# tyb311/TCCT

Measured on AMD Instinct MI355X. Metric: OCT B-scans/sec fwd+bwd(+clip+AdamW), stc_tt bs=8 1x800x1100, higher is better.
Workload: dtype bf16; 1 GPU; stc_tt --los=di bs=8/GPU 1x800x1100 (net tensors 3x800x1104); global_batch=8, parallelism=dp1, ranks=1, grad_allreduce=none, slowest_step=101

## Files before the change

### include/tcct_hip.h

```cpp
#ifndef TCCT_HIP_H
#define TCCT_HIP_H
#include <stdint.h>
#ifdef __cplusplus
extern "C" {
#endif

typedef void* tcct_stream_t;

enum { TCCT_F32 = 0, TCCT_BF16 = 1 };
enum { TCCT_ACT_NONE = 0, TCCT_ACT_LRELU = 1, TCCT_ACT_HSWISH = 2, TCCT_ACT_GELU = 3, TCCT_ACT_SIGMOID = 4,
       TCCT_ACT_ABS = 5 };

int tcct_version(void);
const char* tcct_last_error(void);
int tcct_set_outputs_prezeroed(int on);

int tcct_image_to_nhwc4(const float* img, void* out, int N, int Csrc, int H, int Wsrc, int Wdst, int dtype,
                        tcct_stream_t stream);
int tcct_u8_gather2d(const uint8_t* src, uint8_t* dst, int N, int SH, int SW, int C, int sy0, int sx0, int sh, int sw, int DH, int DW,
                     int dy0, int dx0, int dh, int dw, int flipy, int flipx, int mul, int div, int fill, tcct_stream_t stream);
int tcct_onehot_to_index(const int64_t* onehot, uint8_t* lab, int N, int C, int64_t HW, tcct_stream_t stream);
int tcct_labels_to_u8(const int64_t* lab, uint8_t* out, int N, int H, int Wsrc, int Wdst, tcct_stream_t stream);
int tcct_nhwc_to_nchw_f32(const void* x, float* y, int N, int64_t HW, int C, int dtype, tcct_stream_t stream);

// ... 50 lines not shown
int tcct_bn2_add_act_train(const void* xa, const void* xb, void* y, int64_t M, int C, const double* sumsA, const float* gammaA,
                           const float* betaA, float* running_meanA, float* running_varA, int64_t* nbtA, float* mean_rstdA,
                           float* abA, const double* sumsB, const float* gammaB, const float* betaB, float* running_meanB,
                           float* running_varB, int64_t* nbtB, float* mean_rstdB, float* abB, float eps, float momentum,
                           int pre_act, int act, int dtype, tcct_stream_t stream);
int tcct_bn2_add_act_bwd_reduce(const void* xa, const void* xb, const void* dy, int64_t M, int C, const float* mean_rstdA,
                                const float* abA, const float* mean_rstdB, const float* abB, int pre_act, int act, double* sums,
                                int dtype, tcct_stream_t stream);
int tcct_bn2_add_act_bwd_apply(const void* xa, const void* xb, const void* dy, void* dxa, void* dxb, int64_t M, int C,
                               const float* mean_rstdA, const float* abA, const float* mean_rstdB, const float* abB,
                               const double* sums, int pre_act, int act, float* dgammaA, float* dbetaA, float* dgammaB,
                               float* dbetaB, int dtype, tcct_stream_t stream);

int tcct_layernorm_fwd(const void* x, void* y, int64_t M, int C, const float* gamma, const float* beta, float eps,
                       float* mean_rstd , int dtype, tcct_stream_t stream);
int tcct_layernorm_bwd(const void* x, const void* dy, void* dx, int64_t M, int C, const float* gamma,
                       const float* mean_rstd, float* dgamma, float* dbeta, int dtype, tcct_stream_t stream);
int tcct_layernorm_bwd_add(const void* x, const void* dy, const void* res, void* dx, int64_t M, int C, const float* gamma,
                           const float* mean_rstd, float* dgamma, float* dbeta, int dtype, tcct_stream_t stream);

int tcct_conv2d_fwd(const void* x, const float* w, const float* bias, void* y, int N, int H, int W, int Cin,
                    int Cin_w, int Cout, int KH, int KW, int stride, int padh, int padw, int in_dtype, int out_dtype,
                    tcct_stream_t stream);
int tcct_conv2d_dgrad(const void* dy, const float* w, void* dx, int N, int H, int W, int Cin, int Cout, int KH,
                      int KW, int padh, int padw, int dy_dtype, int dx_dtype, tcct_stream_t stream);
int tcct_conv2d_wgrad(const void* x, const void* dy, float* dw, float* dbias, int N, int H, int W, int Cin,
                      int Cin_w, int Cout, int KH, int KW, int stride, int padh, int padw, int x_dtype, int dy_dtype,
                      tcct_stream_t stream);

int tcct_conv32f_pack_weights(const float* w, float* wp, int KH, int KW, int transposed, tcct_stream_t stream);
int tcct_conv32f_fwd(const float* x, const float* wp, const float* bias, const float* yadd, float* y, int N, int H, int W, int KH, int KW, int PH,
                     int PW, tcct_stream_t stream);
int tcct_conv32f_wgrad(const float* x, const float* dy, float* dw, float* dbias, int N, int H, int W, int KH, int KW, int PH, int PW,
                       tcct_stream_t stream);
int tcct_conv32f_pack_weights_sub(const float* w, float* wp, int KH, int KW, int transposed, int cin_total, int o_off, int i_off, tcct_stream_t stream);
int tcct_conv32f_fwd_strided(const float* x, const float* wp, const float* bias, float* y, int N, int H, int W, int KH, int KW, int PH, int PW, int xs,
                             int xo, int ys, int yo, int accumulate, tcct_stream_t stream);
int tcct_conv32f_wgrad_strided(const float* x, const float* dy, float* dw, float* dbias, int N, int H, int W, int KH, int KW, int PH, int PW, int xs,
                               int xo, int ds, int dof, int ldi, int o_off, int i_off, tcct_stream_t stream);
int tcct_pwf_fwd(const float* x, const float* w, const float* bias, float* y, int64_t M, int K, int N, int transposed, tcct_stream_t stream);
int tcct_pwf_wgrad(const float* x, const float* dy, float* dw, float* dbias, int64_t M, int K, int N, tcct_stream_t stream);
int tcct_conv32_pack_weights(const float* w, void* wp, int KH, int KW, int transposed, tcct_stream_t stream);
int tcct_conv32_pack_weights_multi(const void* desc, int n, tcct_stream_t stream);
int tcct_conv32_pack_weights_both(const float* w, void* wp2, int KH, int KW, tcct_stream_t stream);
int tcct_conv32_fwd(const void* x, const void* wp, const float* bias, void* y, int N, int H, int W, int KH, int KW, int PH,
                    int PW, tcct_stream_t stream);

int tcct_conv32_fwd_bnstats(const void* x, const void* wp, const float* bias, void* y, int N, int H, int W, int KH, int KW, int PH,
                            int PW, double* stats, int pre_act, tcct_stream_t stream);
int tcct_conv32_fwd_affine(const void* x, const void* wp, const float* bias, void* y, int N, int H, int W, int KH, int KW,
                           int PH, int PW, const float* ab, int pre_act, int post_act, tcct_stream_t stream);
int tcct_pw_fwd_affine(const void* x, const float* w, const float* bias, void* y, int64_t M, int K, int N, const float* ab,
                       int pre_act, int post_act, int out_dtype, tcct_stream_t stream);
int tcct_pw_fwd_affine_residual(const void* x, const float* w, const float* bias, const float* ab, const void* res, void* y, int64_t M, int K, int N,
                                tcct_stream_t stream);
int tcct_pw_fwd_cat2_affine(const void* x1, const void* x2, const float* w, const float* bias, const float* ab, int post_act, void* y, int64_t M, int K, int N,
                            tcct_stream_t stream);
int tcct_pw_fwd_xaff_affine_residual(const void* y_prev, const float* ab_prev, const float* w, const float* bias, const float* ab, const void* res, void* y,
                                     int64_t M, int K, int N, tcct_stream_t stream);
int tcct_conv32_fwd_add(const void* x, const void* wp, const float* bias, const void* res, void* y, int N, int H, int W, int KH, int KW,
                        int PH, int PW, tcct_stream_t stream);
int tcct_conv32_chain33(const void* x, const void* wp1, const float* bias1, void* mid, const void* wp2, const float* bias2, void* y,
                        const void* res, int N, int H, int W, double* stats, tcct_stream_t stream);
int tcct_conv32_pack_weights_sub(const float* w, void* wp, int KH, int KW, int transposed, int cin_total, int o_off, int i_off,
                                 tcct_stream_t stream);
int tcct_conv32_fwd_strided(const void* x, const void* wp, const float* bias, void* y, int N, int H, int W, int KH, int KW, int PH,
                            int PW, int xs, int xo, int ys, int yo, int accumulate, tcct_stream_t stream);
int tcct_conv32_fwd_strided_bnstats(const void* x, const void* wp, const float* bias, void* y, int N, int H, int W, int KH, int KW, int PH,
                                    int PW, int xs, int xo, int ys, int yo, int accumulate, double* stats, int pre_act, tcct_stream_t stream);
int tcct_conv32_fwd_strided_affine(const void* x, const void* wp, const float* bias, void* y, int N, int H, int W, int KH, int KW, int PH, int PW, int xs,
                                   int xo, int ys, int yo, const float* ab, int pre_act, int post_act, tcct_stream_t stream);
int64_t tcct_conv32_wgrad_mode(int mode);
int64_t tcct_conv32_fwd_mode(int mode);
int tcct_conv32_wgrad_strided(const void* x, const void* dy, float* dw, float* dbias, int N, int H, int W, int KH, int KW, int PH,
                              int PW, int xs, int xo, int ds, int dof, int cin_total, int o_off, int i_off, tcct_stream_t stream);
int tcct_conv32_wgrad(const void* x, const void* dy, float* dw, float* dbias, int N, int H, int W, int KH, int KW, int PH,
                      int PW, tcct_stream_t stream);
int tcct_conv32_bwd3x3(const void* x, const void* dy, const void* wp_t, const void* dskip, void* dx, float* dw, float* dbias, int N, int H,
                       int W, tcct_stream_t stream);

int tcct_pw_fwd(const void* x, const float* w, const float* bias, void* y, int64_t M, int K, int N, int transposed,
                int out_dtype, tcct_stream_t stream);
int tcct_pw_wgrad(const void* x, const void* dy, float* dw, float* dbias, int64_t M, int K, int N, tcct_stream_t stream);
int tcct_pw_bwd(const void* x, const void* dy, const float* w, const void* res, void* dx, float* dw, float* dbias, int64_t M, int K, int N,
                tcct_stream_t stream);
int tcct_pw_bwd_cat2(const void* x1, const void* x2, const void* dy, const float* w, void* dx1, void* dx2, float* dw, int64_t M, int K, int N,
                     tcct_stream_t stream);
int tcct_pw_bwd_residual2(const void* x, const void* dy, const float* w, const void* res, void* dx_sum, void* dx_plain, float* dw, float* dbias,
                          int64_t M, int K, int N, tcct_stream_t stream);
int64_t tcct_pw_bwd_bn_supported(int K, int N, int post, int red_post, int split);
int tcct_pw_bwd_bn(const void* x, const void* x2, const void* dz, const void* y, const float* coef, int post, const float* w, const void* res,
                   void* dx, void* dx2, float* dw, float* dbias, int64_t M, int K, int N, const void* y_prev, const float* ab_prev,
                   int red_post, double* sums_prev, tcct_stream_t stream);
int tcct_pw_bwd_bn_sums(const void* x, const void* x2, const void* dz, const void* y, const double* sums, int raw, const float* mean_rstd,
                        const float* ab, float* dgamma, float* dbeta, int post, const float* w, const void* res, void* dx, void* dx2, float* dw,
                        float* dbias, int64_t M, int K, int N, const void* y_prev, const float* ab_prev, int red_post, double* sums_prev,
                        tcct_stream_t stream);
int tcct_pw_wgrad_strided(const void* x, const void* dy, int64_t ldy, float* dw, float* dbias, int64_t M, int K, int N,
                          tcct_stream_t stream);
int tcct_pw_fwd_residual(const void* x, const float* w, const float* bias, const void* res, const float* scale, int64_t per_sample,
                         void* y, void* y_plain, int64_t M, int K, int N, tcct_stream_t stream);
int tcct_pw_fwd_bnstats_xaff(const void* y_prev, const float* ab_prev, const float* w, const float* bias, void* y, int64_t M, int K, int N, double* stats,
                             tcct_stream_t stream);
int tcct_pw_bwd_bn_sums_xaff(const void* y_prev, const float* ab_prev, const void* dz, const void* y, const double* sums, int raw, const float* mean_rstd,
                             const float* ab, float* dgamma, float* dbeta, const float* w, const void* res, void* dx, float* dw, float* dbias, int64_t M,
                             int K, int N, int red_post, double* sums_prev, tcct_stream_t stream);
int tcct_pw_fwd_gelu_residual(const void* x1, const float* w, const float* bias, const void* res, const float* scale, int64_t per_sample, void* y,
                              int64_t M, int K, int N, tcct_stream_t stream);
int tcct_pw_bwd_residual2_sum(const void* x, const void* dy_a, const void* dy_b, const float* w, const void* res, void* dx_sum, void* dx_plain, float* dw,
                              float* dbias, int64_t M, int K, int N, tcct_stream_t stream);
int tcct_pw_bwd_lnb(const void* x, const void* dy, const float* w, const void* t, const float* mean_rstd, const float* gamma, const void* res, void* dt,
                    float* dw, float* dbias, float* dgamma, float* dbeta, int64_t M, int K, int N, tcct_stream_t stream);
int tcct_pw_bwd_gelu(const void* x1, const void* dy, const float* w, void* dx1, float* dw, float* dbias, int64_t M, int K, int N, tcct_stream_t stream);
int tcct_pw_dgrad_residual(const void* dy, const float* w, const void* res, void* dx_sum, void* dx_plain, int64_t M, int Nout, int K,
                           tcct_stream_t stream);
int tcct_pw_fwd_cat2(const void* x1, const void* x2, int K1, const float* w, const float* bias, void* y, int64_t M, int K, int N,
                     double* stats, int pre_act, tcct_stream_t stream);
int tcct_pw_fwd_f32_upadd(const void* x, const float* w, const float* bias, float* y, int B, int uH, int uW, int K, int N, const float* up, tcct_stream_t stream);
int tcct_pw_dgrad_split2(const void* dy, const float* w, void* dx1, void* dx2, int K1, int64_t M, int Nout, int K, tcct_stream_t stream);
int tcct_pw_bwd_cat2_bias(const void* x1, const void* x2, const void* dy, const float* w, void* dx1, void* dx2, float* dw, float* dbias, int64_t M,
                          int K, int N, tcct_stream_t stream);
int tcct_tail_compose(const float* w1, const float* b1, const float* w2, const float* b2, float* wc, float* c, tcct_stream_t stream);
int tcct_tail_compose_bwd(const float* w1, const float* b1, const float* w2, const float* dwc, const float* dc, float* dw1, float* db1, float* dw2,
                          float* db2, tcct_stream_t stream);
int tcct_tail_compose3(const float* w1, const float* b1, const float* w2, const float* b2, const float* w3, const float* b3, int C, float* wcc, float* wa,
                       float* wb, float* ccc, tcct_stream_t stream);
int tcct_tail_compose3_bwd(const float* w1, const float* b1, const float* w2, const float* b2, const float* w3, int C, const float* dwa, const float* dwb,
                           const float* dccc, float* dw1, float* db1, float* dw2, float* db2, float* dw3, float* db3, tcct_stream_t stream);
int tcct_pw_fwd_cat2_f32(const void* x1, const void* x2, int K1, const float* w, const float* bias, float* y, int64_t M, int K, int N, tcct_stream_t stream);
int tcct_head_compose(const float* wt, const float* bt, const float* wa, const float* ba, int C, float* wh, float* ch, tcct_stream_t stream);
int tcct_head_compose_bwd(const float* wt, const float* bt, const float* wa, int C, const float* dwh, const float* dch, float* dwt, float* dbt,
                          float* dwa, float* dba, tcct_stream_t stream);
int tcct_pw_wgrad_cat2(const void* x1, const void* x2, int K1, const void* dy, float* dw, float* dbias, int64_t M, int K, int N,
                       tcct_stream_t stream);
int tcct_pw_fwd_bnstats(const void* x, const float* w, const float* bias, void* y, int64_t M, int K, int N, double* stats, int pre_act,
                        tcct_stream_t stream);

int tcct_im2col3x3_c3(const void* x4, void* out, int N, int H, int W, int stride, int dtype, tcct_stream_t stream);
int tcct_c3_fwd(const void* x4, const float* w, const float* bias, void* y, int B, int H, int W, int stride, double* stats, int stat_pre,
                const float* ab, int pre_act, int post_act, tcct_stream_t stream);
int tcct_c3_wgrad(const void* x4, const void* dy, float* dw, float* dbias, int B, int H, int W, int stride, tcct_stream_t stream);
int tcct_c3_bn_fwd_train(const void* x4, const float* w, const float* bias, void* z, int B, int H, int W, int stride, double* sums,
                         const float* gamma, const float* beta, float eps, float momentum, float* running_mean, float* running_var,
                         int64_t* num_batches_tracked, float* mean_rstd, float* ab, int post_act, tcct_stream_t stream);
int tcct_c3_bn_fwd_eval(const void* x4, const float* w, const float* bias, void* z, int B, int H, int W, int stride, const float* ab, int post_act,
                        tcct_stream_t stream);
int tcct_c3_bn_bwd_reduce(const void* x4, const float* w, const float* bias, const void* dz, int B, int H, int W, int stride, const float* ab,
                          double* raw, int post_act, tcct_stream_t stream);
int tcct_c3_bn_bwd_wgrad(const void* x4, const float* w, const float* bias, const void* dz, int B, int H, int W, int stride, const float* coef,
                         float* dw, float* dbias, int post_act, tcct_stream_t stream);
int64_t tcct_c3_bn_bwd_prefetch(int tiles_ahead);
int tcct_c3_bn_bwd_onepass(const void* x4, const float* w, const float* bias, const void* dz, int B, int H, int W, int stride, const float* mean_rstd,
                           const float* ab, float* work, double* sums, float* dw, float* dbias, float* dgamma, float* dbeta, int post_act, tcct_stream_t stream);
int tcct_pw_wgrad_smalln(const void* x, const void* dy, float* dw, float* dbias, int64_t M, int K, int N, int x_dtype,
                         int dy_dtype, tcct_stream_t stream);

int tcct_stream_copy(const void* src, void* dst, int64_t nbytes, tcct_stream_t stream);

int64_t tcct_kernel_census(int which, int reset);
int tcct_marker(int id, tcct_stream_t stream);

int tcct_dwconv3x3_fwd(const void* x, const float* w, const float* bias, void* y, int N, int H, int W, int C,
                       int stride, int add_input, int dtype, tcct_stream_t stream);
int tcct_dwconv3x3_fwd_bnstats(const void* x, const float* w, const float* bias, void* y, int N, int H, int W, int C, int stride,
                               int add_input, double* stats, int dtype, tcct_stream_t stream);
int tcct_dwconv3x3_dgrad(const void* dy, const float* w, void* dx, int N, int H, int W, int C, int stride,
// ... 123 lines not shown
```

### tcct_amd/_lib.py

```python
import ctypes
import threading
import os
import re

import torch

_HERE = os.path.dirname(os.path.abspath(__file__))
LIB_PATH = os.path.join(_HERE, 'csrc', 'libtcct_hip.so')
if os.environ.get('TCCT_LIB_PATH'):
    LIB_PATH = os.path.abspath(os.environ['TCCT_LIB_PATH'])
HEADER = os.path.join(_HERE, '..', 'include', 'tcct_hip.h')

F32, BF16 = 0, 1
ACT_NONE, ACT_LRELU, ACT_HSWISH, ACT_GELU, ACT_SIGMOID, ACT_ABS = range(6)

_CT = {'int': ctypes.c_int, 'int64_t': ctypes.c_int64, 'float': ctypes.c_float, 'double': ctypes.c_double,
       'uint64_t': ctypes.c_uint64}


def parse_header(path=HEADER):
    src = open(path).read()
    src = re.sub(r'/\*.*?\*/', ' ', src, flags=re.S)
    src = re.sub(r'//[^\n]*', ' ', src)
    protos = {}
    for m in re.finditer(r'(const\s+char\s*\*|int64_t|int)\s+(tcct_\w+)\s*\(([^)]*)\)\s*;', src):
        ret, name, args = m.group(1), m.group(2), m.group(3).strip()
        sig = []
        if args and args != 'void':
            for a in args.split(','):
                a = ' '.join(a.split())
                if '*' in a or a.startswith('tcct_stream_t'):
                    sig.append((ctypes.c_void_p, a.split()[-1].lstrip('*')))
                else:
                    ty, nm = a.rsplit(' ', 1)
                    sig.append((_CT[ty.replace('const ', '').strip()], nm))
        protos[name] = (ctypes.c_char_p if 'char' in ret else (ctypes.c_int64 if 'int64' in ret else ctypes.c_int), sig)
    return protos


class TcctError(RuntimeError):
    pass


_TLS = threading.local()
_TRACE = [None]


class launch_on:

    def __init__(self, stream):
        self.handle = stream.cuda_stream

    def __enter__(self):
        self.prev = getattr(_TLS, 'stream', None)
        _TLS.stream = self.handle
        return self

    def __exit__(self, *exc):
        _TLS.stream = self.prev
        return False


class _Lib:
    def __init__(self):
        self._dll = None
        self.protos = parse_header()

    def load(self):
        if self._dll is None:
            if not os.path.exists(LIB_PATH):
                raise TcctError(f'{LIB_PATH} is missing: run `python -c "import __graft_entry__ as g; g.build()"` '
                                '(tcct_amd has no CPU fallback)')
            dll = ctypes.CDLL(LIB_PATH)
            for name, (res, sig) in self.protos.items():
                fn = getattr(dll, name)
                fn.restype = res
                fn.argtypes = [t for t, _ in sig]
            self._dll = dll
        return self._dll

    def last_error(self):
        return self.load().tcct_last_error().decode()

    def __getattr__(self, name):
        full = 'tcct_' + name
        if full not in self.protos:
            raise AttributeError(name)
        dll = self.load()
        fn = getattr(dll, full)
        sig = self.protos[full][1]
        res_is_value = self.protos[full][0] is not ctypes.c_int

        n = len(sig)
        has_stream = bool(sig) and sig[-1][1] == 'stream'
        is_ptr = tuple(ct is ctypes.c_void_p for ct, _ in sig)
        raw_stream, cur_dev, Tensor = torch._C._cuda_getCurrentRawStream, torch._C._cuda_getDevice, torch.Tensor

        tls, trace = _TLS, _TRACE

        def call(*args):
            if has_stream and len(args) == n - 1:
                args = args + (getattr(tls, 'stream', None) or raw_stream(cur_dev()),)
            elif len(args) != n:
                raise TypeError(f'{full}: expected {n} args ({[nm for _, nm in sig]}), got {len(args)}')
            if has_stream and trace[0] is not None:
                trace[0](full, sig, args)
            rc = fn(*[(a.data_ptr() if isinstance(a, Tensor) else a) if p and a is not None else a for a, p in zip(args, is_ptr)])
            if res_is_value:
                return rc
            if rc != 0:
                raise TcctError(f'{full} failed (rc={rc}): {dll.tcct_last_error().decode()}')
        call.__name__ = full
        self.__dict__[name] = call
        return call


lib = _Lib()


def dtype_code(t):
    if t == torch.float32:
        return F32
    if t == torch.bfloat16:
        return BF16
    raise TcctError(f'unsupported activation dtype {t}')
```

### tcct_amd/csrc/pw_mfma.hip

```cpp
#include "common.h"
#include "c3_geom.h"
#include <cstdlib>

typedef __attribute__((ext_vector_type(8))) __bf16 bf16x8;
typedef __attribute__((ext_vector_type(16))) float f32x16;
typedef __attribute__((ext_vector_type(4))) short s16x4;
typedef __attribute__((ext_vector_type(8))) short s16x8;
typedef __attribute__((__vector_size__(4 * sizeof(unsigned int)))) unsigned int u32x4;

#define PWB 256

__device__ __forceinline__ void st_out4(bf16* p, float a, float b, float c, float d) {
    uint2 o; o.x = pack_bf16x2(a, b); o.y = pack_bf16x2(c, d);
    *reinterpret_cast<uint2*>(p) = o;
}
__device__ __forceinline__ void st_out4(float* p, float a, float b, float c, float d) {
    *reinterpret_cast<float4*>(p) = make_float4(a, b, c, d);
}

__device__ __forceinline__ float rnd_out(float v, const bf16*) { return __bfloat162float(__float2bfloat16(v)); }
__device__ __forceinline__ float rnd_out(float v, const float*) { return v; }

struct PwUp { const float* p; int uH, uW, Ho, Wo; float sh, sw; uint32_t m_howo, m_wo; };
struct PwSplit { const bf16* x2; int K1; void* y2; int N1; const bf16* res; const float* rscale; int64_t per_sample; bf16* yplain; C3Geom c3; PwUp up; };
// ... 541 lines not shown
        return __builtin_bit_cast(bf16x8, v);
    };
    struct WF { bf16x8 a[NT], b[KTB]; };
    auto load_chunk = [&](WF& f, int ch) {
#pragma unroll
        for (int ct = 0; ct < NT; ++ct) f.a[ct] = tr2(lbD + ch * 16 * SD + 64 * ct, SD);
#pragma unroll
        for (int kt = 0; kt < KTB; ++kt) f.b[kt] = tr2(lbX + ch * 16 * SX + 64 * kt, SX);
    };
    auto mma_chunk = [&](const WF& f) {
        if (blockIdx.y == 0) {
#pragma unroll
            for (int ct = 0; ct < NT; ++ct)
#pragma unroll
                for (int j = 0; j < 8; ++j) bsum[ct] += (float)f.a[ct][j];
        }
#pragma unroll
        for (int kt = 0; kt < KTB; ++kt)
#pragma unroll
            for (int ct = 0; ct < NT; ++ct) acc[ct][kt] = __builtin_amdgcn_mfma_f32_32x32x16_bf16(f.a[ct], f.b[kt], acc[ct][kt], 0, 0, 0);
    };
    const int64_t tiles = (M + PW_P - 1) / PW_P;
    int64_t tile = blockIdx.x;
    if (C3)
        for (int i = tid; i < PW_P * 2; i += PWB) *reinterpret_cast<uint4*>(sX + (i >> 1) * SX + (6 + (i & 1)) * 16) = make_uint4(0, 0, 0, 0);
    if (tile < tiles) prefetch(tile);
    for (; tile < tiles; tile += gridDim.x) {
        __syncthreads();
        if (C3) {
#pragma unroll
            for (int j = 0; j < 3; ++j)
                if (xsl[j] >= 0) *reinterpret_cast<uint4*>(sX + (tid & 127) * SX + (xsl[j] & 255) * 16) = px[j];
        } else
#pragma unroll
        for (int j = 0; j < PW_XS; ++j)
            if (xsl[j] >= 0) *reinterpret_cast<uint4*>(sX + (xsl[j] >> 8) * SX + (xsl[j] & 255) * 16) = px[j];
#pragma unroll
        for (int j = 0; j < DSN; ++j)
            if (dsl[j] >= 0) *reinterpret_cast<uint4*>(sD + (dsl[j] >> 8) * SD + (dsl[j] & 255) * 16) = pd[j];
        __syncthreads();
        if (C3 || tile + gridDim.x < tiles) prefetch(tile + gridDim.x);
        WF f0, f1;
        load_chunk(f0, wave);
        load_chunk(f1, wave + 4);
        __builtin_amdgcn_sched_barrier(0);
        mma_chunk(f0);
        mma_chunk(f1);
        __builtin_amdgcn_sched_barrier(0);
    }
    __syncthreads();
    float* red = reinterpret_cast<float*>(smem);
    for (int turn = 0; turn < 4; ++turn) {
        if (wave == turn) {
#pragma unroll
            for (int ct = 0; ct < NT; ++ct)
#pragma unroll
                for (int kt = 0; kt < KTB; ++kt)
#pragma unroll
                    for (int k = 0; k < 16; ++k) {
                        const int co = ct * 32 + (k & 3) + 8 * (k >> 2) + 4 * hh;
                        float* dst = &red[co * (KTB * 32) + kt * 32 + r];
                        *dst = turn == 0 ? acc[ct][kt][k] : *dst + acc[ct][kt][k];
                    }
        }
        __syncthreads();
    }
    for (int i = tid; i < NT * 32 * KTB * 32; i += PWB) {
        const int co = i / (KTB * 32), cl = i - co * (KTB * 32);
        if (C3) {
            if (cl < 48 && ((cl >> 2) & 3) < 3 && (cl & 3) < 3) atomicAdd(&dw[co * 27 + (cl & 3) * 9 + (cl >> 4) * 3 + ((cl >> 2) & 3)], red[i]);
        }
        else
        if (co < N && ci_base + cl < K) atomicAdd(&dw[(int64_t)co * K + ci_base + cl], red[i]);
    }
    if (dbias && blockIdx.y == 0) {
#pragma unroll
        for (int ct = 0; ct < NT; ++ct) {
            float s = bsum[ct] + __shfl_xor(bsum[ct], 32, 64);
            if (lane < 32 && ct * 32 + r < N) atomicAdd(&dbias[ct * 32 + r], s);
        }
    }
}

static int pw_wgrad_impl(const void* x, const void* x2, int K1, const void* dy, float* dw, float* dbias, int64_t M, int K, int N, tcct_stream_t stream,
                         int64_t ldy);
extern "C" int tcct_pw_wgrad(const void* x, const void* dy, float* dw, float* dbias, int64_t M, int K, int N, tcct_stream_t stream) {
    return pw_wgrad_impl(x, nullptr, 0, dy, dw, dbias, M, K, N, stream, 0);
}
extern "C" int tcct_pw_wgrad_cat2(const void* x1, const void* x2, int K1, const void* dy, float* dw, float* dbias, int64_t M, int K, int N,
                                  tcct_stream_t stream) {
    TCCT_CHECK(x2 != nullptr && K1 % 32 == 0 && K1 > 0 && K1 < K, "pw_wgrad_cat2: K1=%d must be a multiple of 32 inside (0, K)", K1);
    return pw_wgrad_impl(x1, x2, K1, dy, dw, dbias, M, K, N, stream, 0);
}
extern "C" int tcct_pw_wgrad_strided(const void* x, const void* dy, int64_t ldy, float* dw, float* dbias, int64_t M, int K, int N,
                                     tcct_stream_t stream) {
    return pw_wgrad_impl(x, nullptr, 0, dy, dw, dbias, M, K, N, stream, ldy);
}
static int pw_wgrad_impl(const void* x, const void* x2, int K1, const void* dy, float* dw, float* dbias, int64_t M, int K, int N, tcct_stream_t stream,
                         int64_t ldy) {
    if (ldy == 0) ldy = N;
    TCCT_CHECK(ldy >= N && ldy % 8 == 0, "pw_wgrad: ldy=%lld must be a multiple of 8 and >= N=%d", (long long)ldy, N);
    TCCT_CHECK(K % 32 == 0 && N % 32 == 0 && K >= 32 && N >= 32 && N <= 160 && K <= 1024, "pw_wgrad: unsupported K=%d N=%d", K, N);
    hipStream_t st = (hipStream_t)stream;
    if (!tcct_skip_zero_fill() && hipMemsetAsync(dw, 0, sizeof(float) * (size_t)N * K, st) != hipSuccess) { tcct_set_error("pw_wgrad: memset failed"); return -2; }
    if (dbias && !tcct_skip_zero_fill() && hipMemsetAsync(dbias, 0, sizeof(float) * N, st) != hipSuccess) { tcct_set_error("pw_wgrad: memset failed"); return -2; }
    const int NT = N / 32, ktiles = K / 32;
    const int KTB = (ktiles % 2 == 0 && NT <= 2) ? 2 : 1;
    const int gy = ktiles / KTB;
    TCCT_CHECK(!x2 || K1 % (KTB * 32) == 0, "pw_wgrad_cat2: K1=%d must be a multiple of %d for this shape", K1, KTB * 32);
    const int SX = KTB == 1 ? 64 : 192;
    const int SD = 2 * N + ((NT & 1) ? 0 : 64);
    size_t lds = (size_t)PW_P * (SX + SD);
    size_t red = (size_t)NT * 32 * KTB * 32 * 4;
    if (red > lds) lds = red;
    const int64_t tiles = (M + PW_P - 1) / PW_P;
    (void)hipFuncSetAttribute;
    int per_cu = (int)((160 * 1024) / (lds + 512));
    if (per_cu > 2) per_cu = 2;
    if (per_cu < 1) per_cu = 1;
    int gx = 256 * per_cu / gy;
    if (gx < 64) gx = 64;
    if (tiles <= 1024) { int small = 128 / gy; if (small < 16) small = 16; if (gx > small) gx = small; }
    if (gx > tiles) gx = (int)tiles;
    if (gx < 1) gx = 1;
#define WL(NTV, KV) { static bool at_ = false; if (!at_) { (void)hipFuncSetAttribute((const void*)k_pw_wgrad<NTV, KV>, hipFuncAttributeMaxDynamicSharedMemorySize, 160 * 1024); at_ = true; } } hipLaunchKernelGGL((k_pw_wgrad<NTV, KV>), dim3(gx, gy), dim3(PWB), lds, st, (const bf16*)x, (const bf16*)dy, dw, dbias, M, K, N, SX, SD, (const bf16*)x2, K1, ldy)
    if (KTB == 2) { switch (NT) { case 1: WL(1, 2); break; default: WL(2, 2); break; } }
    else { switch (NT) { case 1: WL(1, 1); break; case 2: WL(2, 1); break; case 3: WL(3, 1); break; case 4: WL(4, 1); break; default: WL(5, 1); break; } }
#undef WL
    TCCT_LAUNCH_OK();
}


extern "C" int tcct_c3_wgrad(const void* x4, const void* dy, float* dw, float* dbias, int B, int H, int W, int stride, tcct_stream_t stream) {
    TCCT_CHECK(stride == 1 || stride == 2, "c3_wgrad: stride %d", stride);
    const int Ho = (H - 1) / stride + 1, Wo = (W - 1) / stride + 1;
    const int64_t M = (int64_t)B * Ho * Wo, inb = (int64_t)B * H * W * 8;
    TCCT_CHECK(M > 0 && M * 64 < (1ll << 31) && inb < (1ll << 31), "c3_wgrad: image too large for 32-bit byte offsets (B=%d H=%d W=%d)", B, H, W);
    hipStream_t st = (hipStream_t)stream;
    if (!tcct_skip_zero_fill() && hipMemsetAsync(dw, 0, sizeof(float) * 32 * 27, st) != hipSuccess) { tcct_set_error("c3_wgrad: memset failed"); return -2; }
    if (dbias && !tcct_skip_zero_fill() && hipMemsetAsync(dbias, 0, sizeof(float) * 32, st) != hipSuccess) { tcct_set_error("c3_wgrad: memset failed"); return -2; }
    const int SX = 192, SD = 64;
    const size_t lds = (size_t)PW_P * (SX + SD);
    const int64_t tiles = (M + PW_P - 1) / PW_P;
    int gx = (int)(tiles / 48 < 256 ? 256 : (tiles / 48 > 1024 ? 1024 : tiles / 48));
    if (gx > tiles) gx = (int)tiles;
    auto magic = [](uint32_t d) { return d == 1 ? 0xffffffffu : (uint32_t)((1ull << 32) / d); };
    hipLaunchKernelGGL((k_pw_wgrad<1, 2, true>), dim3(gx, 1), dim3(PWB), lds, st, (const bf16*)x4, (const bf16*)dy, dw, dbias, M, 64, 32, SX, SD,
                       (const bf16*)nullptr, 0, (int64_t)32,
                       C3Geom{H, W, Ho, Wo, stride, (uint32_t)inb, (Wo + 31) / 32, magic((uint32_t)((Wo + 31) / 32)), magic((uint32_t)Ho), magic((uint32_t)(Ho * Wo)), magic((uint32_t)Wo)});
    TCCT_LAUNCH_OK();
}


#define PB_P 128

__device__ __forceinline__ u32x4 gelu8(u32x4 v) {
    u32x4 o;
#pragma unroll
    for (int k = 0; k < 4; ++k)
        o[k] = pack_bf16x2(act_c<TCCT_ACT_GELU>(__uint_as_float(v[k] << 16)), act_c<TCCT_ACT_GELU>(__uint_as_float(v[k] & 0xffff0000u)));
    return o;
}
__device__ __forceinline__ float gelu_grad1(float x) { float c, p; gauss_cdf_pdf(x, c, p); return c + x * p; }
template <int KIND> __device__ __forceinline__ u32x4 affine8(u32x4 v, const float* __restrict__ a, const float* __restrict__ b) {
    const float4 a0 = *reinterpret_cast<const float4*>(a), a1 = *reinterpret_cast<const float4*>(a + 4);
    const float4 b0 = *reinterpret_cast<const float4*>(b), b1 = *reinterpret_cast<const float4*>(b + 4);
    const float aa[8] = {a0.x, a0.y, a0.z, a0.w, a1.x, a1.y, a1.z, a1.w}, bb[8] = {b0.x, b0.y, b0.z, b0.w, b1.x, b1.y, b1.z, b1.w};
    u32x4 o;
#pragma unroll
    for (int k = 0; k < 4; ++k)
        o[k] = pack_bf16x2(act_c<KIND>(aa[2 * k] * __uint_as_float(v[k] << 16) + bb[2 * k]),
                           act_c<KIND>(aa[2 * k + 1] * __uint_as_float(v[k] & 0xffff0000u) + bb[2 * k + 1]));
    return o;
}
struct PwBnBwd { const bf16* y; const float* coef; const bf16* yprev; const float* abprev; double* sums_prev;
                 const double* sums; int raw; const float* mean_rstd; const float* ab; float* dgamma; float* dbeta; };
template <int KIND> __device__ __forceinline__ float pw_act_grad(float u) {
    if (KIND == TCCT_ACT_HSWISH) return u < -3.f ? 0.f : (u <= 3.f ? (2.f * u + 3.f) * (1.f / 6.f) : 1.f);
    return 1.f;
}
template <int NT, int KT, bool SPLIT = false, int BNP = -1, int REDP = -1, bool GX = false, int XAP = -1, bool LNB = false, bool DY2 = false>
__global__ void __launch_bounds__(PWB, 2)
k_pw_bwd(const bf16* __restrict__ x, const bf16* __restrict__ dy, const float* __restrict__ w, const bf16* __restrict__ res,
         bf16* __restrict__ dx, bf16* __restrict__ dx_plain, float* __restrict__ dw, float* __restrict__ dbias, int64_t M, PwBnBwd bn) {
    constexpr int K = 32 * KT, N = 32 * NT;
    constexpr bool BN = BNP >= 0, RED = REDP >= 0;
    constexpr int SX = 64 * KT + ((KT & 1) ? 0 : 64), SD = 64 * NT + ((NT & 1) ? 0 : 64);
    constexpr int SW = 2 * N + 16;
    constexpr int XS = K / 16, DS = N / 16;
    extern __shared__ __attribute__((aligned(16))) unsigned char smem[];
    unsigned char* sX = smem;
    unsigned char* sD = sX + PB_P * SX;
    unsigned char* sW = sD + PB_P * SD;
    unsigned char* sS = sW + ((K * SW + 15) & ~15);
    float* sC = reinterpret_cast<float*>(sS + 4 * 2560);
    float* sP = sC + (BN ? 5 * N : 0);
    const int tid = threadIdx.x, lane = tid & 63, wave = tid >> 6;
    const int r = lane & 31, hh = lane >> 5;
    for (int i = tid; i < N * K; i += PWB) {
        const int n = i / K, k = i - n * K;
        *reinterpret_cast<bf16*>(sW + k * SW + n * 2) = __float2bfloat16(w[i]);
    }
    if (BN) {
        if (bn.coef) { for (int i = tid; i < 5 * N; i += PWB) sC[i] = bn.coef[i]; }
        else if (tid < N) {
            const int c = tid;
            const double mu = bn.mean_rstd[c], rs = bn.mean_rstd[N + c];
// ... 1006 lines not shown
```

### tcct_amd/ops.py

```python
import os
import weakref

import torch

from ._lib import lib, dtype_code, TcctError, launch_on, F32, BF16

ACT = {None: 0, 'none': 0, 'lrelu': 1, 'hswish': 2, 'gelu': 3, 'sigmoid': 4, 'abs': 5}


class _ZeroPool:

    def __init__(self):
        self.buf = None
        self.off = 0
        self.active = False
        self.frozen = False

    def begin(self, device, nbytes=8 << 20):
        if self.buf is None or self.buf.device != device or self.buf.numel() < nbytes:
            if self.frozen:
                raise TcctError('the zero pool cannot be re-allocated after a training step was captured into a hipGraph '
                                f'(pool on {self.buf.device}, step on {device})')
            self.buf = torch.empty(nbytes, device=device, dtype=torch.uint8)
        self.buf.zero_()
        self.off = 0
        self.active = True
        lib.set_outputs_prezeroed(1)

    def end(self):
        if self.active:
            self.active = False
            lib.set_outputs_prezeroed(0)

    def get(self, shape, dtype, device):
        n = 1
        for d in shape:
            n *= d
        nbytes = n * dtype.itemsize
        if not self.active:
            return torch.empty(shape, device=device, dtype=dtype)
        start = (self.off + 255) // 256 * 256
        if self.buf.device != device or start + nbytes > self.buf.numel():
            return torch.zeros(shape, device=device, dtype=dtype)
        self.off = start + nbytes
        return self.buf[start:start + nbytes].view(dtype).view(shape)


ZERO = _ZeroPool()


PACK_ALL = True
_PACKS = {'ent': {}, 'desc': None, 'sig': None, 'fresh': False, 'step': 0, 'frozen': False, 'keep': []}


def packs_freeze():
    _PACKS['frozen'] = True
    if _PACKS['desc'] is not None:
        _PACKS['keep'].append((_PACKS['desc'], [e[1] for e in _PACKS['ent'].values()]))


def _pack_lookup(w, KH, KW):
    if not (PACK_ALL and ZERO.active):
        return None
    ent = _PACKS['ent'].get(id(w))
    if ent is None or ent[0]() is not w or ent[3] != w.data_ptr() or ent[2] != (KH, KW):
        wp2 = torch.empty(2 * KH * KW * 1024, device=w.device, dtype=torch.bfloat16)
        _PACKS['ent'][id(w)] = [weakref.ref(w), wp2, (KH, KW), w.data_ptr(), _PACKS['step']]
        _PACKS['sig'] = None
        return None
    ent[4] = _PACKS['step']
    if not _PACKS['fresh'] or _PACKS['sig'] is None or not ent[5:]:
        return None
    n = KH * KW * 1024
    return ent[1][:n], ent[1][n:]


def _pack_evict():
    step = _PACKS['step']
    for k in [k for k, e in _PACKS['ent'].items() if e[0]() is None or e[0]().data_ptr() != e[3] or e[4] < step]:
        del _PACKS['ent'][k]
    _PACKS['step'] = step + 1


def _pack_all(device):
    ents = [e for e in _PACKS['ent'].values() if e[0]().device == device]
    _PACKS['fresh'] = False
    if not (PACK_ALL and ents):
        return
# ... 109 lines not shown
    raise TcctError('fresh_stream: no stream of the pool is free of aliases')


class _wgrad_stream:
    def __init__(self, enable, *tensors):
        self.enable, self.tensors = enable, tensors

    def __enter__(self):
        if not self.enable:
            return self
        cur = torch.cuda.current_stream()
        key = ('wgrad', cur.device.index)
        ent = _SIDE_STREAMS.get(key)
        if ent is None:
            ent = _SIDE_STREAMS[key] = (fresh_stream(cur.device), torch.cuda.Event())
        self.side, ev = ent
        if _WGRAD_FRESH_EVENT:
            ev = torch.cuda.Event()
        ev.record(cur)
        self.side.wait_event(ev)
        self.ctx = launch_on(self.side)
        self.ctx.__enter__()
        return self

    def __exit__(self, *exc):
        if not self.enable:
            return False
        self.ctx.__exit__(*exc)
        if _WGRAD_RECORD_STREAM:
            for t in self.tensors:
                t.record_stream(self.side)
        else:
            _WGRAD_KEEP.extend(self.tensors)
        _WGRAD_USED[id(self.side)] = self.side
        return False


def _slot_written(*params):
    return PARALLEL_BRANCHES and ZERO.active and all(p is None or getattr(p, '_grad_slot', None) is not None for p in params)


def _grad_out(param, shape=None):
    slot = getattr(param, '_grad_slot', None)
    if slot is not None and ZERO.active:
        return slot.view(shape if shape is not None else slot.shape)
    return ZERO.get(tuple(shape if shape is not None else param.shape), torch.float32, param.device)


def _ret(t, param):
    if t is None:
        return None
    slot = getattr(param, '_grad_slot', None)
    if slot is not None and t.data_ptr() == slot.data_ptr():
        return None
    return t


def _chk(*ts):
    for t in ts:
        if t is None:
            continue
        if not t.is_cuda:
            raise TcctError('tcct_amd ops need CUDA(HIP) tensors; there is no CPU fallback')
        if not t.is_contiguous():
            raise TcctError(f'non-contiguous tensor of shape {tuple(t.shape)} passed to a HIP op')


def _c(t):
    return t if t.is_contiguous() else t.contiguous()


def _as(t, dtype):
    t = _c(t)
    return t if t.dtype == dtype else t.to(dtype)


def _mfma32_ok(in_dt, out_dt, Cin, Cin_w, Cout, KH, KW, stride, padh, padw):
    return (in_dt == torch.bfloat16 and out_dt == torch.bfloat16 and Cin == 32 and Cin_w == 32 and Cout == 32 and stride == 1
            and 2 * padh == KH - 1 and 2 * padw == KW - 1 and KH * KW > 1 and (KH == 1 or KW == 1 or (KH == 3 and KW == 3)))


F32_MFMA = True
F32_PW = [os.environ.get('TCCT_F32_PW_FWD', '0') == '1', True, True]


def _mfma32f_ok(in_dt, out_dt, Cin, Cin_w, Cout, KH, KW, stride, padh, padw):
    return (F32_MFMA and in_dt == torch.float32 and out_dt == torch.float32 and Cin == 32 and Cin_w == 32 and Cout == 32 and stride == 1
            and 2 * padh == KH - 1 and 2 * padw == KW - 1 and 1 < KH * KW <= 13 and (KH == 1 or KW == 1 or (KH == 3 and KW == 3)))


def _pwf_ok(in_dt, out_dt, Cin, Cin_w, Cout, KH, KW, stride, padh, padw):
    return (F32_MFMA and in_dt == torch.float32 and out_dt == torch.float32 and KH == 1 and KW == 1 and stride == 1 and padh == 0 and padw == 0
            and Cin == Cin_w and Cin % 32 == 0 and Cout % 32 == 0)


def _mfma_slabs_ok(in_dt, out_dt, Cin, Cin_w, Cout, KH, KW, stride, padh, padw):
    return (in_dt == torch.bfloat16 and out_dt == torch.bfloat16 and Cin == Cin_w and Cin % 32 == 0 and Cout % 32 == 0
            and 32 <= Cin <= 256 and 32 <= Cout <= 256 and (Cin, Cout) != (32, 32) and stride == 1
            and 2 * padh == KH - 1 and 2 * padw == KW - 1 and KH * KW > 1 and max(KH, KW) <= 13
            and (KH == 1 or KW == 1 or (KH == 3 and KW == 3)))


def _mfma_slabs_f32_ok(in_dt, out_dt, Cin, Cin_w, Cout, KH, KW, stride, padh, padw):
    return (F32_MFMA and in_dt == torch.float32 and out_dt == torch.float32 and Cin == Cin_w and Cin % 32 == 0 and Cout % 32 == 0
            and 32 <= Cin <= 256 and 32 <= Cout <= 256 and (Cin, Cout) != (32, 32) and stride == 1
            and 2 * padh == KH - 1 and 2 * padw == KW - 1 and 1 < KH * KW <= 13 and (KH == 1 or KW == 1 or (KH == 3 and KW == 3)))


def _conv_slabs_fwd_f32(x, w, bias, y, N, H, W, Cin, Cout, KH, KW, padh, padw, transposed):
    for oh in range(Cout // 32):
        for ih in range(Cin // 32):
            wp = torch.empty(KH * KW * 1024, device=x.device, dtype=torch.float32)
            if not transposed:
                lib.conv32f_pack_weights_sub(w, wp, KH, KW, 0, Cin, 32 * oh, 32 * ih)
            else:
                lib.conv32f_pack_weights_sub(w, wp, KH, KW, 1, Cout, 32 * ih, 32 * oh)
            b = bias[32 * oh:32 * oh + 32] if (bias is not None and ih == 0) else None
            lib.conv32f_fwd_strided(x, wp, b, y, N, H, W, KH, KW, padh, padw, Cin, 32 * ih, Cout, 32 * oh, 1 if ih > 0 else 0)


def _conv_slabs_fwd(x, w, bias, y, N, H, W, Cin, Cout, KH, KW, padh, padw, transposed, stats=None, stat_pre=0):
    wp = torch.empty(KH * KW * 1024, device=x.device, dtype=torch.bfloat16)
    for oh in range(Cout // 32):
        for ih in range(Cin // 32):
            if not transposed:
                lib.conv32_pack_weights_sub(w, wp, KH, KW, 0, Cin, 32 * oh, 32 * ih)
            else:
                lib.conv32_pack_weights_sub(w, wp, KH, KW, 1, Cout, 32 * ih, 32 * oh)
            b = bias[32 * oh:32 * oh + 32] if (bias is not None and ih == 0) else None
            if stats is not None and ih == Cin // 32 - 1:
                lib.conv32_fwd_strided_bnstats(x, wp, b, y, N, H, W, KH, KW, padh, padw, Cin, 32 * ih, Cout, 32 * oh, 1 if ih > 0 else 0, stats, stat_pre)
            else:
                lib.conv32_fwd_strided(x, wp, b, y, N, H, W, KH, KW, padh, padw, Cin, 32 * ih, Cout, 32 * oh, 1 if ih > 0 else 0)
            if ih + 1 < Cin // 32 or oh + 1 < Cout // 32:
                wp = torch.empty_like(wp)


FUSED_CONV_BWD = False
FUSED_PW_BWD = True


def _pw_bwd_ok(x, dy, Cin, Cin_w, Cout, KH, KW, stride, padh, padw):
    return (x.dtype == torch.bfloat16 and dy.dtype == torch.bfloat16 and KH == 1 and KW == 1 and stride == 1 and padh == 0 and padw == 0
            and Cin == Cin_w and Cin % 32 == 0 and Cout % 32 == 0 and 32 <= Cin <= 128 and 32 <= Cout <= 128
            and x.numel() * 2 < 2 ** 31 and dy.numel() * 2 < 2 ** 31)


def _pw_ok(in_dt, Cin, Cin_w, KH, KW, stride, padh, padw):
    return (in_dt == torch.bfloat16 and KH == 1 and KW == 1 and stride == 1 and padh == 0 and padw == 0 and Cin == Cin_w
            and Cin % 32 == 0)


class _Conv2d(_FastFunction):
    @staticmethod
    def forward(ctx, x, w, bias, stride, padh, padw, out_dtype, stats_box, fork=False):
        ctx.set_materialize_grads(False)
        _chk(x, w, bias)
        N, H, W, Cin = x.shape
        Cout, Cin_w, KH, KW = w.shape
        Ho = (H + 2 * padh - KH) // stride + 1
        Wo = (W + 2 * padw - KW) // stride + 1
        odt = out_dtype or x.dtype
        y = torch.empty((N, Ho, Wo, Cout), device=x.device, dtype=odt)
        mfma = _mfma32_ok(x.dtype, odt, Cin, Cin_w, Cout, KH, KW, stride, padh, padw)
        if _pw_ok(x.dtype, Cin, Cin_w, KH, KW, stride, padh, padw) and not mfma:
            if stats_box is not None and odt == torch.bfloat16 and Cout % 32 == 0 and Cout <= 160:
# ... 2622 lines not shown
```

Before: 420.4 B-scans/s.

## Add single-pass pointwise weight-gradient kernel covering all K tiles per block

Adds a new pointwise-conv weight-gradient kernel that has each 1024-thread block load a row tile of dy once, together with a wide group of input-channel tiles, and accumulate every (Cin,Cout) 32x32 tile from that shared LDS copy. The existing path splits K across many grid rows and re-reads dy for each. The new kernel also uses register prefetch of the next tile and transposed LDS reads into MFMA. It is enabled by default through a host flag (env-controllable) when there are at least two K-groups, at the cost of lower occupancy (one large block per CU) and more LDS per block.

```diff
diff --git a/include/tcct_hip.h b/include/tcct_hip.h
--- a/include/tcct_hip.h
+++ b/include/tcct_hip.h
@@ -156,6 +156,7 @@
 int tcct_pw_fwd(const void* x, const float* w, const float* bias, void* y, int64_t M, int K, int N, int transposed,
                 int out_dtype, tcct_stream_t stream);
 int tcct_pw_wgrad(const void* x, const void* dy, float* dw, float* dbias, int64_t M, int K, int N, tcct_stream_t stream);
+int tcct_set_pw_wgrad_oneread(int on);
 int tcct_pw_bwd(const void* x, const void* dy, const float* w, const void* res, void* dx, float* dw, float* dbias, int64_t M, int K, int N,
                 tcct_stream_t stream);
 int tcct_pw_bwd_cat2(const void* x1, const void* x2, const void* dy, const float* w, void* dx1, void* dx2, float* dw, int64_t M, int K, int N,
diff --git a/tcct_amd/_lib.py b/tcct_amd/_lib.py
--- a/tcct_amd/_lib.py
+++ b/tcct_amd/_lib.py
@@ -44,6 +44,7 @@
 
 _TLS = threading.local()
 _TRACE = [None]
+ON_LOAD = []
 
 
 class launch_on:
@@ -77,6 +78,8 @@
                 fn.restype = res
                 fn.argtypes = [t for t, _ in sig]
             self._dll = dll
+            for hook in ON_LOAD:
+                hook(dll)
         return self._dll
 
     def last_error(self):
diff --git a/tcct_amd/csrc/pw_mfma.hip b/tcct_amd/csrc/pw_mfma.hip
--- a/tcct_amd/csrc/pw_mfma.hip
+++ b/tcct_amd/csrc/pw_mfma.hip
@@ -647,6 +647,108 @@
     }
 }
 
+#define PWA 1024
+#define PWA_D 3
+#define PWA_X 5
+template <int ACC>
+__global__ void __launch_bounds__(PWA, 1)
+k_pw_wgrad_all(const bf16* __restrict__ x, const bf16* __restrict__ dy, float* __restrict__ dw, float* __restrict__ dbias, int64_t M,
+               int K, int N, int ST, const bf16* __restrict__ x2, int K1, int64_t ldy, int KG) {
+    extern __shared__ __attribute__((aligned(16))) unsigned char smem[];
+    const int tid = threadIdx.x, lane = tid & 63, wave = tid >> 6;
+    const int r = lane & 31, hh = lane >> 5;
+    const int NT = N >> 5, dc = N >> 3;
+    const int ci_base = blockIdx.y * KG * 32;
+    const int kgn = min(KG, (K >> 5) - blockIdx.y * KG);
+    const int ntile = NT * kgn;
+    const int ld1 = x2 ? K1 : K, ld2 = K - K1;
+    const int prow = tid >> 3, pc = tid & 7;
+    const int xc = kgn * 4;
+    uint4 pd[PWA_D], px[PWA_X];
+    auto prefetch = [&](int64_t tile) {
+        const int64_t m = tile * PW_P + prow;
+        const bool in = m < M;
+        const bf16* pdy = dy + m * ldy + pc * 8;
+        const bf16* p1 = x + m * ld1 + ci_base + pc * 8;
+        const bf16* p2 = x2 + m * ld2 + (ci_base - K1) + pc * 8;
+#pragma unroll
+        for (int j = 0; j < PWA_D; ++j) {
+            pd[j] = make_uint4(0, 0, 0, 0);
+            if (in && pc + 8 * j < dc) pd[j] = *reinterpret_cast<const uint4*>(pdy + 64 * j);
+        }
+#pragma unroll
+        for (int j = 0; j < PWA_X; ++j) {
+            px[j] = make_uint4(0, 0, 0, 0);
+            if (in && pc + 8 * j < xc) px[j] = *reinterpret_cast<const uint4*>(((x2 && ci_base + (pc + 8 * j) * 8 >= K1) ? p2 : p1) + 64 * j);
+        }
+    };
+    const int li = lane & 15, lq = li >> 2, lpp = li & 3, lg = lane >> 4;
+    const unsigned char* lb = smem + (8 * (lg >> 1) + lq) * ST + (16 * (lg & 1) + 4 * lpp) * 2;
+    auto tr2 = [&](const unsigned char* p) {
+        s16x4 lo = __builtin_amdgcn_ds_read_tr16_b64_v4i16((__attribute__((address_space(3))) s16x4*)p);
+        s16x4 hi = __builtin_amdgcn_ds_read_tr16_b64_v4i16((__attribute__((address_space(3))) s16x4*)(p + 4 * ST));
+        s16x8 v = __builtin_shufflevector(lo, hi, 0, 1, 2, 3, 4, 5, 6, 7);
+        return __builtin_bit_cast(bf16x8, v);
+    };
+    f32x16 acc[ACC];
+    int ta[ACC], tb[ACC];
+#pragma unroll
+    for (int a = 0; a < ACC; ++a) {
+#pragma unroll
+        for (int k = 0; k < 16; ++k) acc[a][k] = 0.f;
+        const int t = wave + 16 * a, kt = t / NT;
+        ta[a] = 64 * (t - kt * NT); tb[a] = dc * 16 + 64 * kt;
+    }
+    float bsum = 0.f;
+    const bool bias_wave = dbias && blockIdx.y == 0 && wave < NT;
+    const int64_t tiles = (M + PW_P - 1) / PW_P;
+    int64_t tile = blockIdx.x;
+    if (tile < tiles) prefetch(tile);
+    for (; tile < tiles; tile += gridDim.x) {
+        __syncthreads();
+#pragma unroll
+        for (int j = 0; j < PWA_D; ++j)
+            if (pc + 8 * j < dc) *reinterpret_cast<uint4*>(smem + prow * ST + (pc + 8 * j) * 16) = pd[j];
+#pragma unroll
+        for (int j = 0; j < PWA_X; ++j)
+            if (pc + 8 * j < xc) *reinterpret_cast<uint4*>(smem + prow * ST + (dc + pc + 8 * j) * 16) = px[j];
+        __syncthreads();
+        if (tile + gridDim.x < tiles) prefetch(tile + gridDim.x);
+#pragma unroll
+        for (int a = 0; a < ACC; ++a) {
+            if (wave + 16 * a >= ntile) break;
+#pragma unroll 2
+            for (int ch = 0; ch < 8; ++ch) {
+                const bf16x8 fa = tr2(lb + ch * 16 * ST + ta[a]);
+                const bf16x8 fb = tr2(lb + ch * 16 * ST + tb[a]);
+                if (a == 0 && bias_wave) {
+#pragma unroll
+                    for (int j = 0; j < 8; ++j) bsum += (float)fa[j];
+                }
+                acc[a] = __builtin_amdgcn_mfma_f32_32x32x16_bf16(fa, fb, acc[a], 0, 0, 0);
+            }
+        }
+    }
+#pragma unroll
+    for (int a = 0; a < ACC; ++a) {
+        const int t = wave + 16 * a;
+        if (t >= ntile) break;
+        const int kt = t / NT, ct = t - kt * NT;
+#pragma unroll
+        for (int k = 0; k < 16; ++k) {
+            const int co = ct * 32 + (k & 3) + 8 * (k >> 2) + 4 * hh;
+            atomicAdd(&dw[(int64_t)co * K + ci_base + kt * 32 + r], acc[a][k]);
+        }
+    }
+    if (bias_wave) {
+        const float s = bsum + __shfl_xor(bsum, 32, 64);
+        if (lane < 32) atomicAdd(&dbias[wave * 32 + r], s);
+    }
+}
+
+static int g_pw_wgrad_oneread = 1;
+extern "C" int tcct_set_pw_wgrad_oneread(int on) { g_pw_wgrad_oneread = on ? 1 : 0; return 0; }
+
 static int pw_wgrad_impl(const void* x, const void* x2, int K1, const void* dy, float* dw, float* dbias, int64_t M, int K, int N, tcct_stream_t stream,
                          int64_t ldy);
 extern "C" int tcct_pw_wgrad(const void* x, const void* dy, float* dw, float* dbias, int64_t M, int K, int N, tcct_stream_t stream) {
@@ -672,13 +774,12 @@
     const int NT = N / 32, ktiles = K / 32;
     const int KTB = (ktiles % 2 == 0 && NT <= 2) ? 2 : 1;
     const int gy = ktiles / KTB;
-    TCCT_CHECK(!x2 || K1 % (KTB * 32) == 0, "pw_wgrad_cat2: K1=%d must be a multiple of %d for this shape", K1, KTB * 32);
+    const int64_t tiles = (M + PW_P - 1) / PW_P;
     const int SX = KTB == 1 ? 64 : 192;
     const int SD = 2 * N + ((NT & 1) ? 0 : 64);
     size_t lds = (size_t)PW_P * (SX + SD);
     size_t red = (size_t)NT * 32 * KTB * 32 * 4;
     if (red > lds) lds = red;
-    const int64_t tiles = (M + PW_P - 1) / PW_P;
     (void)hipFuncSetAttribute;
     int per_cu = (int)((160 * 1024) / (lds + 512));
     if (per_cu > 2) per_cu = 2;
@@ -688,6 +789,22 @@
     if (tiles <= 1024) { int small = 128 / gy; if (small < 16) small = 16; if (gx > small) gx = small; }
     if (gx > tiles) gx = (int)tiles;
     if (gx < 1) gx = 1;
+    if (g_pw_wgrad_oneread && gy >= 2) {
+        int kgmax = 8 * PWA_X / 4;
+        if (kgmax > 32 / NT) kgmax = 32 / NT;
+        const int gy1 = (ktiles + kgmax - 1) / kgmax, KG = (ktiles + gy1 - 1) / gy1;
+        const int ACC = (NT * KG + 15) / 16;
+        const int ST = (16 * (N / 8 + KG * 4) - 64 + 127) / 128 * 128 + 64;
+        const size_t lds1 = (size_t)PW_P * ST;
+        int gx1 = gx * 5 / 2 < 256 ? gx * 5 / 2 : 256;
+        if (tiles <= 1024) { int small = 128 / gy1; if (small < 16) small = 16; if (gx1 > small) gx1 = small; }
+        if (gx1 > tiles) gx1 = (int)tiles;
+#define WA(AV) { static bool at_ = false; if (!at_) { (void)hipFuncSetAttribute((const void*)k_pw_wgrad_all<AV>, hipFuncAttributeMaxDynamicSharedMemorySize, 160 * 1024); at_ = true; } } hipLaunchKernelGGL((k_pw_wgrad_all<AV>), dim3(gx1, gy1), dim3(PWA), lds1, st, (const bf16*)x, (const bf16*)dy, dw, dbias, M, K, N, ST, (const bf16*)x2, K1, ldy, KG)
+        if (ACC == 1) { WA(1); } else { WA(2); }
+#undef WA
+        TCCT_LAUNCH_OK();
+    }
+    TCCT_CHECK(!x2 || K1 % (KTB * 32) == 0, "pw_wgrad_cat2: K1=%d must be a multiple of %d for this shape", K1, KTB * 32);
 #define WL(NTV, KV) { static bool at_ = false; if (!at_) { (void)hipFuncSetAttribute((const void*)k_pw_wgrad<NTV, KV>, hipFuncAttributeMaxDynamicSharedMemorySize, 160 * 1024); at_ = true; } } hipLaunchKernelGGL((k_pw_wgrad<NTV, KV>), dim3(gx, gy), dim3(PWB), lds, st, (const bf16*)x, (const bf16*)dy, dw, dbias, M, K, N, SX, SD, (const bf16*)x2, K1, ldy)
     if (KTB == 2) { switch (NT) { case 1: WL(1, 2); break; default: WL(2, 2); break; } }
     else { switch (NT) { case 1: WL(1, 1); break; case 2: WL(2, 1); break; case 3: WL(3, 1); break; case 4: WL(4, 1); break; default: WL(5, 1); break; } }
diff --git a/tcct_amd/ops.py b/tcct_amd/ops.py
--- a/tcct_amd/ops.py
+++ b/tcct_amd/ops.py
@@ -3,7 +3,7 @@
 
 import torch
 
-from ._lib import lib, dtype_code, TcctError, launch_on, F32, BF16
+from ._lib import lib, dtype_code, TcctError, launch_on, ON_LOAD, F32, BF16
 
 ACT = {None: 0, 'none': 0, 'lrelu': 1, 'hswish': 2, 'gelu': 3, 'sigmoid': 4, 'abs': 5}
 
@@ -279,6 +279,14 @@
 
 F32_MFMA = True
 F32_PW = [os.environ.get('TCCT_F32_PW_FWD', '0') == '1', True, True]
+PW_WGRAD_ONEREAD = os.environ.get('TCCT_PW_WGRAD_ONEREAD', '1') != '0'
+ON_LOAD.append(lambda dll: dll.tcct_set_pw_wgrad_oneread(int(PW_WGRAD_ONEREAD)))
+
+
+def set_pw_wgrad_oneread(on):
+    global PW_WGRAD_ONEREAD
+    PW_WGRAD_ONEREAD = bool(on)
+    lib.set_pw_wgrad_oneread(int(PW_WGRAD_ONEREAD))
 
 
 def _mfma32f_ok(in_dt, out_dt, Cin, Cin_w, Cout, KH, KW, stride, padh, padw):
```

Result: no change. 422.3 B-scans/s, median of 6 (+0.4%).
